# kouei/ray-tracing-in-one-weekend

Hardware: AMD Instinct MI355X
Metric: Mray/s (ray segments = closest-hit queries per second), final random-spheres scene 3840x2160 @ 500spp depth 50 (higher is better)
Workload: dtype fp32

## Files before the change

include/rt_internal.h:

```cpp
#ifndef RTOW_RT_INTERNAL_H
#define RTOW_RT_INTERNAL_H

#include "rt.h"

#ifdef __cplusplus
extern "C" {
#endif

enum { RT_OPT_INTERNAL_GRID_PHASE_X = 8, RT_OPT_INTERNAL_GRID_PHASE_Z = 9 };

enum { RT_KAT_SPHERE_HIT = 0, RT_KAT_REFLECT = 1, RT_KAT_REFRACT = 2, RT_KAT_REFLECTANCE = 3 };
int rt_device_kat(int device, int kind, const double *in, size_t n_cases, double *out);

#define RT_ACCEL_INFO_N 18
int rt_internal_accel_info(const rt_scene_view *scene, int grid_placement, double grid_scale, uint64_t *out,
                           size_t n_out);

#define RT_LAUNCH_PLAN_N 5
int rt_internal_launch_plan(const rt_params *params, double launch_samples, uint64_t *out, size_t n_out);

int rt_internal_grid_fit(const rt_scene_view *scene, const rt_camera *cam, int width, int height, double *scale,
                         double *costs, size_t n_costs, size_t *n);
int rt_internal_grid_fit_phase(const rt_scene_view *scene, const rt_camera *cam, int width, int height,
                               double phase_x, double phase_z, double *scale, double *costs, size_t n_costs,
                               size_t *n);
int rt_internal_grid_scale(rt_context *ctx, double *scale);

int rt_internal_sealed(const rt_scene_view *scene, uint8_t *out, size_t n_out);

#ifdef __cplusplus
}
#endif
#endif
```

ray-tracing-in-one-weekend_amd/csrc/rt_accel.cpp:

```cpp
#include "rt_accel.h"

#include <algorithm>
#include <cmath>
#include <cstring>
#include <vector>

namespace rtk {
namespace {

struct bvh_builder {
  struct box {
    double lo[3], hi[3];
  };
  std::vector<box> sb;
  std::vector<double> cen;
  std::vector<uint32_t> ord;
  std::vector<bvh_node> nodes;
  std::vector<int> slots;
  static constexpr int kLeaf = 2 * kLeafPairs;
  int max_leaf = kLeaf;
  double collapse_area = 0.35;
  double side_weight = 1.0;
  double grid_phase_x = 0.0, grid_phase_z = 0.0;

// ... 355 lines not shown
}

bool scene_ok(const rt_scene_view *s) {
  if (!s || (s->n && (!s->cx || !s->cy || !s->cz || !s->radius || !s->mat_kind || !s->mat_param ||
                      !s->albedo_rgb)))
    return false;
  for (uint32_t i = 0; i < s->n; ++i) {
    if (s->mat_kind[i] > RT_DIELECTRIC || !(s->radius[i] != 0.0f) || !std::isfinite(s->radius[i]) ||
        !std::isfinite(s->cx[i]) || !std::isfinite(s->cy[i]) || !std::isfinite(s->cz[i]))
      return false;
    for (int k = 0; k < 3 && s->mat_kind[i] != RT_DIELECTRIC; ++k)
      if (!(s->albedo_rgb[3 * i + k] >= 0.0f && std::isfinite(s->albedo_rgb[3 * i + k]))) return false;
  }
  return true;
}

double max_albedo(const rt_scene_view *s) {
  double a = 0.0;
  for (uint32_t i = 0; i < s->n; ++i)
    for (int k = 0; k < 3 && s->mat_kind[i] != RT_DIELECTRIC; ++k) a = std::max(a, (double)s->albedo_rgb[3 * i + k]);
  return a;
}


void build_accel(const rt_scene_view *s, const accel_options &o, accel_build &a, grid_fitter **fitter) {
  if (fitter) *fitter = nullptr;
  const uint32_t n = s->n;
  a = accel_build{};
  a.n = n;
  a.n_pad = (n + kSpherePad - 1) / kSpherePad * kSpherePad;
  a.scan_geom.assign(a.n_pad / 2, pair_geom{});
  for (uint32_t i = 0; i < a.n_pad; ++i) fill_slot(a.scan_geom[i / 2], i & 1, s, i < n ? (int)i : -1);
  a.shade.assign(n, shade_rec{});
  std::vector<uint8_t> sealed;
  sealed_spheres(s, sealed);
  for (uint32_t i = 0; i < n; ++i) {
    shade_rec &r = a.shade[i];
    std::memset(&r, 0, sizeof r);
    r.cx = s->cx[i];
    r.cy = s->cy[i];
    r.cz = s->cz[i];
    r.inv_r = 1.0f / s->radius[i];
    const bool glass = s->mat_kind[i] == RT_DIELECTRIC;
    r.ar = glass ? 1.0f : s->albedo_rgb[3 * i + 0];
    r.ag = glass ? 1.0f : s->albedo_rgb[3 * i + 1];
    r.ab = glass ? 1.0f : s->albedo_rgb[3 * i + 2];
// ... 30 lines not shown
        const double grow = std::max(1.02, 1.01 * std::sqrt((double)need / (double)lds_max));
        if (bb.grid.scale * grow > 1.6 * scale0) break;
        bb.grid.scale *= grow;
        bb.build_grid(s, bb.n_layer);
      }
      if (place != kGridCells && bb.grid.scale != scale0) {
        bb.grid.scale = scale0;
        bb.build_grid(s, bb.n_layer);
      }
    }
  }
  a.bvh_geom.assign(bb.slots.size() / 2, pair_geom{});
  for (size_t k = 0; k < bb.slots.size(); ++k) fill_slot(a.bvh_geom[k / 2], (int)(k & 1), s, bb.slots[k]);
  a.slots = bb.slots;
  a.nodes = bb.nodes;
  a.per_order = bb.per_order;
  a.oref = bb.oref;
  a.layer_mode = bb.layer_mode;
  a.layer_lo = bb.layer_lo;
  a.layer_hi = bb.layer_hi;
  a.layer_cy = bb.layer_cy;
  a.extra_pair0 = bb.extra_pair0;
  a.n_extra_pairs = bb.n_extra_pairs;
  a.grid = bb.grid;
  a.grid_placement = bb.grid.cells.empty() ? kGridGlobal : place;
  if (fitter && !bb.grid.cells.empty())
    *fitter = grid_fitter::make_from(s, o, a.grid_placement, bb.grid.scale, &bb);
}

struct grid_fitter::impl {
  std::vector<float> cx, cy, cz, radius, albedo, param;
  std::vector<uint32_t> kind;
  rt_scene_view view{};
  mutable bvh_builder bb;
  int placement = kGridGlobal;
  size_t lds_max = 0;
  double s0 = 1.0;
  bool grid_at(double scale) const {
    bb.grid.scale = scale;
    bb.build_grid(&view, bb.n_layer);
    if (bb.grid.cells.empty()) return false;
    const long long items = (long long)(bb.grid.items.size() / 4), cells = (long long)bb.grid.cells.size();
    if (placement == kGridLds)
      return items < 4096 && grid_lds_bytes(kGridLds, items, cells) <= lds_max;
    return items < 65536 && grid_lds_bytes(kGridCells, items, cells) <= lds_max;
  }
// ... 107 lines not shown
```

ray-tracing-in-one-weekend_amd/csrc/rt_accel.h:

```cpp
#ifndef RTOW_RT_ACCEL_H
#define RTOW_RT_ACCEL_H

#include <cstdint>
#include <cstring>
#include <vector>

#include "rt_internal.h"
#include "rt_layout.h"

namespace rtk {

struct accel_options {
  int bvh_leaf = 4;
  double collapse = 0.35;
  double side = 1.0;
  double grid_scale = 1.0;
  double grid_phase_x = 0.0, grid_phase_z = 0.0;
  int grid_placement = -1;
  bool wide = false;
};

struct grid_dims {
  float x0 = 0, z0 = 0, xi = 0, zi = 0, x1 = 0, z1 = 0, g = 0;
  int nx = 0, nz = 0;
// ... 4 lines not shown
  }
};
struct grid_geom : grid_dims {
  std::vector<uint32_t> cells;
  std::vector<float> items;
  bool operator==(const grid_geom &o) const {
    return grid_dims::operator==(o) && cells == o.cells && items.size() == o.items.size() &&
           (items.empty() || !std::memcmp(items.data(), o.items.data(), items.size() * sizeof(float)));
  }
};

struct accel_build {
  uint32_t n = 0, n_pad = 0;
  std::vector<pair_geom> scan_geom;
  std::vector<shade_rec> shade;
  std::vector<pair_geom> bvh_geom;
  std::vector<int> slots;
  std::vector<bvh_node> nodes;
  size_t per_order = 0;
  double oref = 64.0;
  bool layer_mode = false;
  float layer_lo = 0.0f, layer_hi = 0.0f, layer_cy = 0.0f;
  uint32_t extra_pair0 = 0, n_extra_pairs = 0;
  grid_geom grid;
  int grid_placement = kGridGlobal;
};

constexpr int kFitSteps = 30;
constexpr double kFitCellCost = 0.5;
class grid_fitter {
 public:
  static grid_fitter *make(const rt_scene_view *s, const accel_options &o, int placement, double scale0);
  ~grid_fitter();
  double choose(const rt_camera &cam, int width, int height, std::vector<std::pair<double, double>> *costs) const;
  bool build(double scale, grid_geom &out) const;
  double scale0() const;
  static grid_fitter *make_from(const rt_scene_view *s, const accel_options &o, int placement, double scale0,
                                void *builder);

 private:
  struct impl;
  impl *p_ = nullptr;
};

bool scene_ok(const rt_scene_view *s);
double max_albedo(const rt_scene_view *s);
void sealed_spheres(const rt_scene_view *s, std::vector<uint8_t> &out);
void build_accel(const rt_scene_view *s, const accel_options &o, accel_build &out, grid_fitter **fitter = nullptr);

}

#endif
```

ray-tracing-in-one-weekend_amd/csrc/rt_aov.hip:

```cpp
#include <hip/hip_runtime.h>

#include <algorithm>
#include <array>
#include <cmath>
#include <cstddef>
#include <cstdint>
#include <cstring>
#include <mutex>
#include <utility>
#include <vector>

#include "rt_aov.h"
#include "rt_device.h"
#include "rt_frame.h"

namespace rtk {

struct aov_params {
  kparams k;
  uint32_t *hits;
  int32_t *id;
  float *depth, *position, *normal, *albedo;
};
static_assert(offsetof(aov_params, k) == 0, "kernargs() reads a kparams at offset 0");
// ... 34 lines not shown
  RT_GLOBAL float *g_alb = as_global(a.albedo);
  const bool first = p.s_lo == 0;
  uint32_t hits = 0;
  int id = -1;
  float dep = 0.0f, sp[3] = {0.0f, 0.0f, 0.0f}, sn[3] = {0.0f, 0.0f, 0.0f}, sa[3] = {0.0f, 0.0f, 0.0f};
  if (!first) {
    if (a.hits) hits = g_hits[o];
    if (a.depth) dep = g_depth[o];
#pragma unroll
    for (int k = 0; k < 3; ++k) {
      if (a.position) sp[k] = g_pos[3 * o + k];
      if (a.normal) sn[k] = g_nrm[3 * o + k];
      if (a.albedo) sa[k] = g_alb[3 * o + k];
    }
  }
  if (grow < p.height) {
    const uint32_t pix = (uint32_t)grow * (uint32_t)p.width + (uint32_t)col;
    work_ctr wc;
    for (int s = p.s_lo; s < p.s_lo + p.s_cnt; ++s) {
      float ox, oy, oz, dx, dy, dz;
      const float tmin = camera_ray(p, pcg4d(pix, (uint32_t)s, 0u, p.seed32), col, grow, ox, oy, oz, dx, dy, dz);
      float walked = 0.0f;
      while (true) {
        const hit_state hs = closest_hit<OPEN, BVH, false, GRID, GP>(ox, oy, oz, dx, dy, dz, tmin, wc);
        const int best = best_of<OPEN>(hs);
        if (best < 0) break;
        const float o2 = dot3(ox, oy, oz, ox, oy, oz);
        const float ox2 = -2.0f * ox, oy2 = -2.0f * oy, oz2 = -2.0f * oz;
        const float tmax = hs.tmax;
        const bool near = near_of(hs) != 0;
        static_assert(sizeof(shade_rec) == 64, "best << 6");
        const shade_rec sr = cload_g((const RT_GLOBAL shade_rec *)((const RT_GLOBAL char *)as_global(p.shade) +
                                                                   ((uint32_t)best << 6)));
        float b;
        const float t = refine_root(sr, tmax, near, ox, oy, oz, dx, dy, dz, o2, ox2, oy2, oz2, b);
        if (b > 0.0f && t < tmin) {
          ox = fmaf(tmax, dx, ox);
          oy = fmaf(tmax, dy, oy);
          oz = fmaf(tmax, dz, oz);
          walked += tmax;
          continue;
        }
        const float px = fmaf(t, dx, ox), py = fmaf(t, dy, oy), pz = fmaf(t, dz, oz);
        const bool front = near != (sr.inv_r < 0.0f);
        const float fir = front ? sr.inv_r : -sr.inv_r;
        const float nx = (px - sr.cx) * fir, ny = (py - sr.cy) * fir, nz = (pz - sr.cz) * fir;
        ++hits;
// ... 175 lines not shown
```

ray-tracing-in-one-weekend_amd/csrc/rt_api.cpp:

```cpp
#include <hip/hip_runtime.h>

#include <algorithm>
#include <cmath>
#include <cstdint>
#include <cstring>
#include <limits>
#include <new>
#include <utility>
#include <vector>

#include "rt_internal.h"
#include "rt_accel.h"
#include "rt_frame.h"
#include "rt_layout.h"

extern "C" hipError_t rt_internal_block_order(const uint32_t *tile_cost, uint32_t blocks, uint32_t units,
                                              uint32_t *order, hipStream_t st);

struct scene_state {
  rtk::pair_geom *d_geom = nullptr;
  rtk::pair_geom *d_bvh_geom = nullptr;
  rtk::bvh_node *d_nodes = nullptr;
  int *d_orig = nullptr;
  rtk::shade_rec *d_shade = nullptr;
  uint32_t n_spheres = 0, n_pad = 0, n_nodes = 0, n_bvh_slots = 0;
  float oref2 = 0.0f;
  bool layer_mode = false;
  float layer_lo = 0.0f, layer_hi = 0.0f, layer_cy = 0.0f;
  uint32_t extra_pair0 = 0, n_extra_pairs = 0;
  uint32_t *d_grid_cells = nullptr;
  float *d_grid_items = nullptr;
  size_t cells_cap = 0, items_cap = 0;
  size_t grid_n_items = 0;
  int grid_placement = rtk::kGridGlobal;
  rtk::grid_dims grid;
  double max_albedo = 0.0;
  rtk::grid_fitter *fitter = nullptr;
  std::vector<uint64_t> fit_key;
  rtk::grid_geom fit_grid;
  bool fit_pending = false;
};

struct rt_context {
  int device = -1;
  hipStream_t stream = nullptr;
  hipEvent_t ev0 = nullptr, ev1 = nullptr;
  scene_state sc;
  hipEvent_t ev_fit = nullptr;
  bool grid_fit = true;
  bool grid_scale_set = false;
  unsigned long long *d_counters = nullptr;
  float *d_frame = nullptr;
// ... 212 lines not shown
      return RT_ERR_INVALID;
  }
}

int rt_scene_upload(rt_context *c, const rt_scene_view *s) {
  if (!c || !rtk::scene_ok(s)) return RT_ERR_INVALID;
  rtk::accel_build a;
  rtk::accel_options o = c->opt;
  o.wide = rtk::max_albedo(s) > 1.0;
  scene_state sc;
  rtk::build_accel(s, o, a, c->grid_fit && !c->grid_scale_set ? &sc.fitter : nullptr);
  sc.n_spheres = a.n;
  sc.max_albedo = rtk::max_albedo(s);
  sc.n_pad = a.n_pad;
  sc.n_nodes = (uint32_t)a.per_order;
  sc.n_bvh_slots = (uint32_t)a.slots.size();
  sc.oref2 = (float)(0.99 * a.oref * a.oref);
  sc.layer_mode = a.layer_mode;
  sc.layer_lo = a.layer_lo;
  sc.layer_cy = a.layer_cy;
  sc.layer_hi = a.layer_hi;
  sc.extra_pair0 = a.extra_pair0;
  sc.n_extra_pairs = a.n_extra_pairs;
  sc.grid = a.grid;

  hipError_t e = hipSetDevice(c->device);
  if (e == hipSuccess && c->have_done) e = hipEventSynchronize(c->ev_done);
  if (e == hipSuccess) e = hipStreamSynchronize(c->stream);
  if (e != hipSuccess) {
    release(sc);
    return hip_fail(e);
  }
  free_scene(c);
  e = upload_vec(&sc.d_geom, a.scan_geom, c->stream);
  if (e == hipSuccess) e = upload_vec(&sc.d_bvh_geom, a.bvh_geom, c->stream);
  if (e == hipSuccess) e = upload_vec(&sc.d_nodes, a.nodes, c->stream);
  if (e == hipSuccess) e = upload_vec(&sc.d_orig, a.slots, c->stream);
  if (e == hipSuccess) e = upload_vec(&sc.d_shade, a.shade, c->stream);
  if (e == hipSuccess && !a.grid.cells.empty()) {
    e = upload_vec(&sc.d_grid_cells, a.grid.cells, c->stream);
    if (e == hipSuccess) e = upload_vec(&sc.d_grid_items, a.grid.items, c->stream);
    sc.cells_cap = a.grid.cells.size();
    sc.items_cap = sc.grid_n_items = a.grid.items.size() / 4;
    sc.grid_placement = a.grid_placement;
  }
  if (e == hipSuccess) e = hipStreamSynchronize(c->stream);
// ... 41 lines not shown
void fill_kparams(const rt_context *c, const rt_camera *cam, const rt_params *prm, float *accum_rgb,
                  rtk::kparams &kp) {
  std::memset(&kp, 0, sizeof kp);
  kp.block_stride = 1;
  kp.cam = *cam;
  kp.width = prm->width;
  kp.height = prm->height;
  kp.spp = prm->spp;
  kp.max_depth = prm->max_depth;
  kp.row_block = prm->row_block;
  kp.band_stride = prm->band_stride;
  kp.band_offset = prm->band_offset;
  kp.local_rows = prm->local_rows;
  kp.tiles_x = (prm->width + rtk::kTile - 1) / rtk::kTile;
  const scene_state &s = c->sc;
  kp.n_pad = (int)s.n_pad;
  kp.n_nodes = (int)s.n_nodes;
  kp.oref2 = s.oref2;
  kp.layer = rtk::f2{s.layer_lo, s.layer_hi};
  kp.layer_mode = s.layer_mode ? 1 : 0;
  kp.layer_cy = s.layer_cy;
  kp.extra_pair0 = (int)s.extra_pair0;
  kp.n_extra_pairs = (int)s.n_extra_pairs;
  grid_kparams(s.grid, s.d_grid_cells, s.d_grid_items, s.grid_n_items, kp);
  kp.seed32 = (uint32_t)prm->seed ^ ((uint32_t)(prm->seed >> 32) * 0x9E3779B9u);
  kp.flags = prm->flags;
  kp.inv_wm1 = (float)(1.0 / (prm->width - 1));
  kp.inv_hm1 = (float)(1.0 / (prm->height - 1));
  kp.scan_geom = s.d_geom;
  kp.geom = s.d_bvh_geom;
  kp.nodes = s.d_nodes;
  kp.orig = s.d_orig;
  kp.extra_geom = s.d_bvh_geom ? s.d_bvh_geom + s.extra_pair0 : nullptr;
  kp.extra_orig = s.d_orig ? s.d_orig + 2 * (size_t)s.extra_pair0 : nullptr;
  kp.shade = s.d_shade;
  kp.out = accum_rgb;
  kp.counters = c->d_counters;
  {
    uint32_t w = (uint32_t)prm->width, sh = 0;
    while (!(w & 1u)) {
      w >>= 1;
      ++sh;
    }
    uint32_t inv = w;
    for (int k = 0; k < 5; ++k) inv *= 2u - w * inv;
    kp.wshift = sh;
    kp.winv = inv;
  }
}

int render_variant(const rt_context *c, const rt_params *prm, bool wide) {
  const bool grid = c->sc.d_grid_cells && !(prm->flags & RT_FLAG_LAYER_BVH);
  const int place = grid ? c->sc.grid_placement : rtk::kGridGlobal;
  return (wide ? rtk::kVarWide : 0) | ((prm->flags & RT_FLAG_OPEN_INTERVAL) ? rtk::kVarOpen : 0) |
         ((prm->flags & RT_FLAG_METAL_UNIT_VECTOR) ? rtk::kVarMetalUnit : 0) |
         ((prm->flags & RT_FLAG_ACCEL_BVH) ? rtk::kVarBvh : 0) |
         ((prm->flags & RT_FLAG_COUNT_WORK) ? rtk::kVarStats : 0) | (grid ? rtk::kVarGrid : 0) |
         (place << rtk::kVarPlaceShift);
}

struct launch_plan {
  long long units, ranges, chunks, entries;
};
launch_plan plan_launches(const rt_params *prm, double launch_samples) {
  const long long tiles = rt_frame_tiles(prm), blocks = rt_frame_blocks(prm);
  const bool traced = prm->spp > 0 && prm->max_depth > 0;
  const double frame_px = (double)prm->width * (double)prm->local_rows;
  const double total = traced ? frame_px * prm->spp : 0.0;
  const double budget = std::max(launch_samples, total / (double)rtk::kMaxLaunches);
  long long units = prm->units;
  if (units <= 0) {
    const bool pilot = (prm->flags & RT_FLAG_PILOT_SCHEDULE) != 0;
    units = pilot ? std::llround((double)rtk::kPilotTilesPerUnit / (double)std::max(1LL, tiles))
                  : (tiles < rtk::kSplitTiles ? rtk::kUnits : 1);
    units = std::min<long long>(std::max(units, 1LL), rtk::kUnits);
  }
  if (!traced) units = 1;
// ... 362 lines not shown
  v[7] = items;
  v[8] = cells ? rtk::grid_lds_bytes(a.grid_placement, (long long)items, (long long)cells) : 0u;
  v[9] = cells && a.grid_placement == rtk::kGridLds;
  uint64_t maxc = 0, listed = 0;
  bool start_ok = true, ring_ok = true;
  for (uint64_t i = 0; i < cells; ++i) {
    const uint32_t first = g.cells[i] >> 4, cnt = g.cells[i] & 15u;
    const uint64_t next = i + 1 < cells ? (g.cells[i + 1] >> 4) : items;
    start_ok = start_ok && first + cnt == next;
    maxc = std::max<uint64_t>(maxc, cnt);
    listed += cnt ? 1u : 0u;
    const int x = (int)(i % g.nx), z = (int)(i / g.nx);
    if (x == 0 || z == 0 || x == g.nx - 1 || z == g.nz - 1) ring_ok = ring_ok && cnt == 0;
  }
  v[10] = maxc;
  v[11] = cells ? (start_ok ? 1u : 0u) : 0u;
  v[12] = cells ? (ring_ok ? 1u : 0u) : 0u;
  v[13] = (uint64_t)(a.oref * 1000.0);
  v[14] = a.layer_mode ? (uint64_t)(2 * a.extra_pair0) : 0u;
  v[15] = listed;
  static const uint64_t kPlaceOut[3] = {RT_GRID_GLOBAL, RT_GRID_LDS, RT_GRID_CELLS_LDS};
  v[16] = cells ? kPlaceOut[a.grid_placement] : 0u;
  v[17] = (uint64_t)std::llround(g.scale * 1000.0);
  std::memcpy(out, v, std::min<size_t>(n_out, RT_ACCEL_INFO_N) * sizeof(uint64_t));
  return RT_OK;
}

int rt_internal_grid_fit(const rt_scene_view *s, const rt_camera *cam, int width, int height, double *scale,
                         double *costs, size_t n_costs, size_t *n) {
  return rt_internal_grid_fit_phase(s, cam, width, height, 0.0, 0.0, scale, costs, n_costs, n);
}

int rt_internal_grid_fit_phase(const rt_scene_view *s, const rt_camera *cam, int width, int height, double phase_x,
                               double phase_z, double *scale, double *costs, size_t n_costs, size_t *n) {
  if (!rtk::scene_ok(s) || !cam || !scale || width < 1 || height < 1 || (n_costs && !costs)) return RT_ERR_INVALID;
  if (!(phase_x >= 0.0 && phase_x < 1.0 && phase_z >= 0.0 && phase_z < 1.0)) return RT_ERR_INVALID;
  rtk::accel_options o;
  o.grid_phase_x = phase_x;
  o.grid_phase_z = phase_z;
  o.wide = rtk::max_albedo(s) > 1.0;
  rtk::accel_build a;
  rtk::grid_fitter *f = nullptr;
  rtk::build_accel(s, o, a, &f);
  *scale = 0.0;
  if (n) *n = 0;
  if (!f) return RT_OK;
// ... 60 lines not shown
```

ray-tracing-in-one-weekend_amd/csrc/rt_device.h:

```cpp
#ifndef RTOW_RT_DEVICE_H
#define RTOW_RT_DEVICE_H

#include <hip/hip_runtime.h>

#include <cstdint>

#include "rt_internal.h"
#include "rt_layout.h"
#include "rt_turn_table.h"

namespace rtk {

#ifndef RT_COUNT_ITEMS
#define RT_COUNT_ITEMS 0
#endif

enum {
  kLpStep = 0, kLpClosest, kLpExtrasLead, kLpExtrasRound, kLpGridWalk, kLpDda, kLpItem, kLpGridCand,
  kLpSky, kLpHit, kLpLamb, kLpMetal, kLpDiel, kLpCamera, kLpSkip, kLpTail, kLpRegions
};
#ifdef RT_LANE_PROFILE
__device__ unsigned long long g_lane_prof[kLpRegions * 3];
__shared__ uint32_t s_lane_prof[4][kLpRegions][3];
__device__ __forceinline__ void lane_prof(int r, bool useful) {
// ... 244 lines not shown
    const f2 gg = fma2(q[j].cz, r.oz2, fma2(q[j].cx, r.ox2, gy));
    e[j] = fma2(h[j], h[j], -gg);
    c[2 * j] = e[j].x >= q[j].ks.x;
    c[2 * j + 1] = e[j].y >= q[j].ks.y;
  }
#pragma unroll
  for (int j = 0; j < 2 * NP; ++j) any |= __builtin_amdgcn_ballot_w64(c[j]);
  if (any) {
    if (STATS) {
#pragma unroll
      for (int j = 0; j < 2 * NP; ++j) roots += __builtin_amdgcn_ballot_w64(c[j]) != 0 ? 1u : 0u;
    }
#pragma unroll
    for (int j = 0; j < NP; ++j) {
      const int s0 = slot0 + 2 * j;
      const int i0 = orig ? orig[s0] : s0;
      const int i1 = orig ? orig[s0 + 1] : s0 + 1;
      if (c[2 * j]) candidate<OPEN>(true, h[j].x, e[j].x - q[j].ks.x, tie2_of<OPEN>((uint32_t)i0), tmin, hs);
      if (c[2 * j + 1]) candidate<OPEN>(true, h[j].y, e[j].y - q[j].ks.y, tie2_of<OPEN>((uint32_t)i1), tmin, hs);
    }
  }
}

template <bool OPEN, bool STATS, bool LEAD>
__device__ __forceinline__ void scan_extras(const RT_CONST pair_geom *__restrict__ g, int slot0,
                                            const RT_CONST int *__restrict__ orig, const ray_pre &r,
                                            float tmin, hit_state &hs, uint32_t &roots) {
  float h[4], d[4];
  uint32_t t[4];
  bool c[4];
#pragma unroll
  for (int j = 0; j < 2; ++j) {
    const pair_geom q = cload(g + j);
#pragma unroll
    for (int s = 0; s < 2; ++s) {
      const float cx = s ? q.cx.y : q.cx.x, cy = s ? q.cy.y : q.cy.x, cz = s ? q.cz.y : q.cz.x;
      const float ks = s ? q.ks.y : q.ks.x;
      const float hy = fmaf(cy, r.dy.x, r.nk1.x);
      const float gy = fmaf(cy, r.oy2.x, r.o2.x);
      const float hh = fmaf(cz, r.dz.x, fmaf(cx, r.dx.x, hy));
      const float gg = fmaf(cz, r.oz2.x, fmaf(cx, r.ox2.x, gy));
      const float ee = fmaf(hh, hh, -gg);
      const int k = 2 * j + s;
      h[k] = hh;
      d[k] = ee - ks;
      c[k] = ee >= ks;
      t[k] = tie2_of<OPEN>((uint32_t)orig[slot0 + k]);
    }
  }
  constexpr int J0 = LEAD ? 1 : 0;
  if (LEAD) {
    if (__builtin_amdgcn_ballot_w64(c[0])) {
      LP(kLpExtrasLead, c[0]);
      if (STATS) ++roots;
      candidate<OPEN>(c[0], h[0], d[0], t[0], tmin, hs);
    }
  }
#pragma unroll
  for (int round = J0; round < 4; ++round) {
    float hh = h[3], dd = d[3];
    uint32_t tt = t[3];
#pragma unroll
    for (int j = 2; j >= J0; --j)
      if (c[j]) {
        hh = h[j];
        dd = d[j];
// ... 156 lines not shown
        ke = k + (ce & 15u);
      }
      uint32_t ko = k << 4;
      const uint32_t koe = ke << 4;
      if (ko != koe) do {
        grid_item<OPEN, STATS>(*(const RT_GLOBAL f4 *)((const RT_GLOBAL char *)items + ko), dx, dz, rl, tmin, hs,
                               wc);
        ko += 16;
      } while (ko != koe);
    }
    const bool sx = tmx < tmz;
    const float tnext = sx ? tmx : tmz;
    float lim;
    asm("v_min_f32 %0, %1, %2" : "=v"(lim) : "v"(tb), "v"(hs.tmax));
    const bool stop = tnext > lim;
    cell += sx ? dcx : dcz;
    tmx = sx ? tmx + tdx : tmx;
    tmz = sx ? tmz : tmz + tdz;
    asm volatile("" : "+v"(cell), "+v"(tmx), "+v"(tmz));
    if (stop) break;
  }
}

template <bool OPEN, bool BVH, bool STATS, bool GRID, int GP>
__device__ __forceinline__ hit_state closest_hit(float ox, float oy, float oz, float dx, float dy, float dz,
                                                 float tmin, work_ctr &wc) {
  const kparams p = kernargs();
  const RT_CONST pair_geom *__restrict__ scan_geom = as_const(p.scan_geom);
  const RT_CONST pair_geom *__restrict__ geom = as_const(p.geom);
  const RT_CONST bvh_node *__restrict__ nodes = as_const(p.nodes);
  const RT_CONST int *__restrict__ orig = as_const(p.orig);
  const int n_pairs = p.n_pad / 2;
  LP(kLpClosest, true);
  const float nk1 = -dot3(ox, oy, oz, dx, dy, dz);
  const float o2 = dot3(ox, oy, oz, ox, oy, oz);
  const float ox2 = -2.0f * ox, oy2 = -2.0f * oy, oz2 = -2.0f * oz;
  hit_state hs = no_hit();
  auto splat = [&]() {
    return ray_pre{{dx, dx}, {dy, dy}, {dz, dz}, {nk1, nk1}, {o2, o2}, {ox2, ox2}, {oy2, oy2}, {oz2, oz2}};
  };
  const bool scan_all = !BVH || __builtin_amdgcn_ballot_w64(o2 > p.oref2) != 0;
  if (scan_all) {
    const ray_pre rp = splat();
    for (int k = 0; k < n_pairs; k += 4)
      scan_pairs<OPEN, 4, STATS>(scan_geom + k, 2 * k, nullptr, rp, tmin, hs, wc.roots);
    if (STATS) wc.tests += 2 * n_pairs;
  } else {
    const ray_pre rp = splat();
    const float ix = __builtin_amdgcn_fmed3f(__builtin_amdgcn_rcpf(dx), -1e18f, 1e18f);
    const float iy = __builtin_amdgcn_fmed3f(__builtin_amdgcn_rcpf(dy), -1e18f, 1e18f);
    const float iz = __builtin_amdgcn_fmed3f(__builtin_amdgcn_rcpf(dz), -1e18f, 1e18f);
    const float oix = -ox * ix, oiy = -oy * iy, oiz = -oz * iz;
    auto walk_order = [&]() {
      const uint32_t half = __builtin_popcountll(__builtin_amdgcn_ballot_w64(true)) / 2;
      const int oct = (__builtin_popcountll(__builtin_amdgcn_ballot_w64(dx < 0.0f)) > half ? 1 : 0) |
                      (__builtin_popcountll(__builtin_amdgcn_ballot_w64(dy < 0.0f)) > half ? 2 : 0) |
                      (__builtin_popcountll(__builtin_amdgcn_ballot_w64(dz < 0.0f)) > half ? 4 : 0);
      return nodes + (size_t)oct * p.n_nodes;
    };
    const RT_CONST bvh_node *__restrict__ order = GRID ? nullptr : walk_order();
    if (GRID || p.layer_mode) {
      if (GRID) {
        const RT_CONST pair_geom *__restrict__ xg = as_const(p.extra_geom);
        const RT_CONST int *__restrict__ xo = as_const(p.extra_orig);
        if (p.n_extra_pairs > 0) scan_extras<OPEN, STATS, true>(xg, 0, xo, rp, tmin, hs, wc.roots);
        for (int k = 2; k < p.n_extra_pairs; k += 2)
          scan_extras<OPEN, STATS, false>(xg + k, 2 * k, xo, rp, tmin, hs, wc.roots);
      } else {
        for (int k = 0; k < p.n_extra_pairs; k += 2)
          scan_pairs<OPEN, 2, STATS>(geom + p.extra_pair0 + k, 2 * (p.extra_pair0 + k), orig, rp, tmin, hs,
                                     wc.roots);
      }
      if (STATS) wc.tests += 2 * p.n_extra_pairs;
      const f2 tyl = fma2(p.layer, f2{iy, iy}, f2{oiy, oiy});
      const float tyl_n = fmaxf(fminf(tyl.x, tyl.y), 0.0f);
      const float tyl_f = fmaxf(tyl.x, tyl.y);
      float tyl_fc = fminf(tyl_f, hs.tmax);
      if (GRID) {
        ray_pre rg = rp;
        rg.nk1.x = fmaf(p.layer_cy, dy, nk1);
        rg.o2.x = fmaf(p.layer_cy, oy2, o2);
        if (tyl_n <= tyl_fc) grid_walk<OPEN, STATS, GP>(ox, oz, ix, iz, oix, oiz, tyl_n, tyl_fc, rg, tmin, hs, wc);
        return hs;
      }
      int node = __builtin_amdgcn_ballot_w64(tyl_n <= tyl_fc) ? 0 : p.n_nodes;
      const f2 vi = {ix, iz}, vo = {oix, oiz}, va = {fabsf(ix), fabsf(iz)};
      ray_pre rl = rp;
      rl.nk1 = fma2(f2{p.layer_cy, p.layer_cy}, rp.dy, rp.nk1);
// ... 35 lines not shown
```

ray-tracing-in-one-weekend_amd/csrc/rt_kernel.hip:

```cpp
#include <hip/hip_runtime.h>

#include <algorithm>
#include <array>
#include <cmath>
#include <cstdint>
#include <type_traits>
#include <utility>

#include "rt_internal.h"
#include "rt_layout.h"
#include "rt_turn_table.h"
#include "rt_device.h"

namespace rtk {


template <bool OPEN, bool METAL_UNIT, bool BVH, bool STATS, bool GRID, int GP, bool WIDE>
__global__ __launch_bounds__(kBlock, 8) void render_kernel(const kparams p) {
  typedef typename std::conditional<WIDE, unsigned long long, uint32_t>::type sum_t;
  const int wave = __builtin_amdgcn_readfirstlane((int)threadIdx.x) >> 6;
  const unsigned entry = blockIdx.x * (unsigned)p.block_stride + (unsigned)p.block_base;
  const unsigned bid = p.block_order ? as_const(p.block_order)[entry] : entry;
  const int unit = (int)(bid % (unsigned)p.units);
  const int tile = (int)(bid / (unsigned)p.units) * kWavesPerBlock + wave;
  const int col0 = (tile % p.tiles_x) * kTile, lrow0 = (tile / p.tiles_x) * kTile;
  const uint32_t s_begin = (uint32_t)p.s_lo + (uint32_t)((uint64_t)unit * (uint32_t)p.s_cnt / (uint32_t)p.units);
  const uint32_t s_end = (uint32_t)p.s_lo + (uint32_t)((uint64_t)(unit + 1) * (uint32_t)p.s_cnt / (uint32_t)p.units);
  const uint32_t kend = (s_end > s_begin ? s_end - s_begin : 0u) << 6;
  __shared__ sum_t s_sum[3][kBlock];
  typedef uint32_t u2v __attribute__((ext_vector_type(2)));
  __shared__ u2v s_rowpix[kWavesPerBlock][kTile];
  {
    const int lane = lane_now();
    const int col = col0 + (lane & (kTile - 1));
    const int lrow = lrow0 + (lane >> 3);
    const int band = lrow / p.row_block;
    const int grow = (band * p.band_stride + p.band_offset) * p.row_block + (lrow - band * p.row_block);
    (void)col;
    if ((lane & (kTile - 1)) == 0) {
      const bool row_in = lrow < p.local_rows && grow < p.height;
// ... 38 lines not shown
    const u2v e = ((const __attribute__((address_space(3))) u2v *)(uintptr_t)rowpix_v)[slot >> 3];
    pix = e.x + (slot & (kTile - 1));
    return (slot & (kTile - 1)) < e.y;
  };
  auto pixel_cr = [&](const kparams &k, int &col, int &grow) {
    col = col0 + (int)(slot & (kTile - 1));
    grow = (int)(((pix - (uint32_t)col) >> k.wshift) * k.winv);
  };
  uint32_t knext = 64;
  bool alive = kend != 0 && p.max_depth > 0;
  bool tracing = false;
  if (alive) {
    tracing = take((uint32_t)lane_now());
    if (tracing) {
      int col, grow;
      pixel_cr(p, col, grow);
      tmin = camera_ray(p, pcg4d(pix, sample, 0u, p.seed32), col, grow, ox, oy, oz, dx, dy, dz);
    }
  }

  while (alive) {
    LP(kLpStep, tracing);
    hit_state hs = no_hit();
    if (tracing) hs = closest_hit<OPEN, BVH, STATS, GRID, GP>(ox, oy, oz, dx, dy, dz, tmin, wc);
    ++steps;
    const int best = best_of<OPEN>(hs);
    const bool miss = !tracing || best < 0;
    uint32_t kn;
    {
      const uint64_t need = __builtin_amdgcn_ballot_w64(miss);
      kn = knext + __builtin_amdgcn_mbcnt_hi((uint32_t)(need >> 32), __builtin_amdgcn_mbcnt_lo((uint32_t)need, 0u));
      knext += (uint32_t)__builtin_popcountll(need);
    }
    bool path_done = false;
    bool skipped = false;
    {
      const kparams q = kernargs();
      if (tracing) ++segs;
      if (tracing && best < 0) {
        LP(kLpSky, true);
        const float a = 0.5f * (dy + 1.0f);
        const float s0 = 1.0f - a;
        const int i = wave * 64 + (int)slot;
        float xr = thr * fmaf(a, 0.5f, s0), xg = thg * fmaf(a, 0.7f, s0), xb = thb * (s0 + a);
        if (WIDE) {
          xr = fminf(xr, q.vcap);
          xg = fminf(xg, q.vcap);
// ... 279 lines not shown
  __shared__ T thr[256];
  thr[threadIdx.x] = thr_g[threadIdx.x];
  __syncthreads();
  const uint64_t n4 = n / 4;
  const bool vec = ((uintptr_t)sums % 16 == 0) && ((uintptr_t)out % 4 == 0);
  const uint64_t stride = (uint64_t)gridDim.x * 256u;
  if (vec) {
    for (uint64_t i = (uint64_t)blockIdx.x * 256u + threadIdx.x; i < n4; i += stride) {
      const f4 v = reinterpret_cast<const f4 *>(sums)[i];
      reinterpret_cast<uint32_t *>(out)[i] =
          tone_level<FP32, T>(v.x, scale, thr) | tone_level<FP32, T>(v.y, scale, thr) << 8 |
          tone_level<FP32, T>(v.z, scale, thr) << 16 | tone_level<FP32, T>(v.w, scale, thr) << 24;
    }
  }
  for (uint64_t i = (vec ? 4 * n4 : 0) + (uint64_t)blockIdx.x * 256u + threadIdx.x; i < n; i += stride)
    out[i] = (uint8_t)tone_level<FP32, T>(sums[i], scale, thr);
}

template <int V>
void launch_variant(unsigned blocks, size_t lds, hipStream_t st, const kparams &kp) {
  constexpr bool O = V & kVarOpen, U = V & kVarMetalUnit, B = V & kVarBvh, S = V & kVarStats;
  constexpr bool G = B && (V & kVarGrid), W = V & kVarWide;
  constexpr int P = G ? ((V >> kVarPlaceShift) & 3) % 3 : kGridGlobal;
  render_kernel<O, U, B, S, G, P, W><<<blocks, kBlock, G ? lds : 0, st>>>(kp);
}
using launch_fn = void (*)(unsigned, size_t, hipStream_t, const kparams &);
template <int... V>
constexpr auto launch_table(std::integer_sequence<int, V...>) {
  return std::array<launch_fn, sizeof...(V)>{&launch_variant<V>...};
}
constexpr auto kLaunch = launch_table(std::make_integer_sequence<int, 2 * kVarWide>{});

hipError_t launch_render(int variant, unsigned blocks, size_t lds_bytes, hipStream_t st, const kparams &kp) {
  if (variant < 0 || variant >= (int)kLaunch.size()) return hipErrorInvalidValue;
  kLaunch[variant](blocks, lds_bytes, st, kp);
  return hipGetLastError();
}

hipError_t launch_finish_sums(uint32_t *frame, uint64_t n, float qinv, hipStream_t st) {
  const unsigned grid = (unsigned)std::min<uint64_t>((n + 255) / 256, 256u * 64u);
  finish_sums<<<grid, 256, 0, st>>>(frame, n, qinv);
  return hipGetLastError();
}

hipError_t launch_finish_sums_wide(const uint64_t *sums, float *frame, uint64_t n, float qinv, hipStream_t st) {
  const unsigned grid = (unsigned)std::min<uint64_t>((n + 255) / 256, 256u * 64u);
  finish_sums_wide<<<grid, 256, 0, st>>>(sums, frame, n, qinv);
  return hipGetLastError();
}

hipError_t launch_tonemap(bool fp32, const float *sums, uint64_t n, int spp, const void *thresholds,
                          uint8_t *out, hipStream_t st) {
  const unsigned grid = (unsigned)std::min<uint64_t>((n / 4 + 255) / 256 + 1, 256u * 32u);
  if (!fp32)
// ... 30 lines not shown
```

ray-tracing-in-one-weekend_amd/csrc/rt_layout.h:

```cpp
#ifndef RTOW_RT_LAYOUT_H
#define RTOW_RT_LAYOUT_H

#include <hip/hip_runtime.h>

#include <cstddef>
#include <cstdint>

#include "rt_internal.h"

namespace rtk {

constexpr int kTile = 8;
constexpr int kWavesPerBlock = 4;
constexpr int kBlock = 64 * kWavesPerBlock;
constexpr int kSpherePad = 8;
constexpr long long kSplitTiles = 12LL * 256 * 4 * 7;
constexpr long long kPilotTilesPerUnit = 16LL * 256 * 4 * 8;
constexpr int kUnits = 8;
constexpr int kCounterSlots = 32;
constexpr double kLaunchSamples = 34359738368.0;
constexpr double kMinPoolSpp = 100.0;
constexpr double kPoolSpp = 250.0;
constexpr long long kMaxLaunches = 65536;

// ... 5 lines not shown
};

struct __attribute__((aligned(32))) bvh_node {
  f2 bx, by, bz;
  int32_t skip;
  uint32_t leaf;
};
constexpr int kLeafPairs = 2;
constexpr uint32_t kTwoPairs = 1u << 31;

struct __attribute__((aligned(16))) shade_rec {
  float cx, cy, cz, inv_r;
  float ar, ag, ab, param;
  uint32_t kind;
  float radius, ks;
  float inv_param;
  float r0;
  uint32_t sealed;
  float pad1, pad2;
};

enum { kGridGlobal = 0, kGridLds = 1, kGridCells = 2 };

struct kparams {
  rt_camera cam;
  int width, height, spp, max_depth;
  int row_block, band_stride, band_offset, local_rows;
  int tiles_x, n_pad, n_nodes;
  float oref2;
  f2 layer;
  int layer_mode, extra_pair0, n_extra_pairs;
  float layer_cy;
  uint32_t seed32, flags;
  float inv_wm1, inv_hm1;
  uint32_t wshift, winv;
  int units, s_lo, s_cnt;
  int sum_atomic;
  float qscale, qinv;
  int dither, block_base;
  int block_stride;
  float vcap;
  const struct pair_geom *scan_geom;
  const struct pair_geom *geom;
  const struct bvh_node *nodes;
  const int *orig;
  const struct shade_rec *shade;
  float *out;
  unsigned long long *counters;
  const uint32_t *block_order;
  uint32_t *tile_cost;
  const uint32_t *grid_cells;
  const f4 *grid_items;
  float grid_x0, grid_z0;
  float grid_xi, grid_zi;
  float grid_x1, grid_z1, grid_g, grid_invg;
  int grid_nx, grid_nz;
  int grid_n_items, grid_n_cells;
  const struct pair_geom *extra_geom;
  const int *extra_orig;
};

__host__ __device__ constexpr size_t grid_lds_bytes(int placement, long long n_items, long long n_cells) {
  return placement == kGridLds ? (size_t)n_items * 16u + ((size_t)(n_cells + 1) * 2u + 15u) / 16u * 16u
         : placement == kGridCells ? ((size_t)(n_cells + 1) * 2u + 15u) / 16u * 16u
                                   : 0u;
}
constexpr size_t kStaticLds = 3 * kBlock * 4 + kWavesPerBlock * kTile * 8;
constexpr size_t kGridLdsMax = 160 * 1024 / 8 - kStaticLds;
constexpr size_t kGridLdsMaxWide = kGridLdsMax - 3 * kBlock * 4;

enum {
  kVarOpen = 1,
  kVarMetalUnit = 2,
  kVarBvh = 4,
  kVarStats = 8,
  kVarGrid = 16,
  kVarPlaceShift = 5,
  kVarWide = 128
};
hipError_t launch_render(int variant, unsigned blocks, size_t lds_bytes, hipStream_t st, const kparams &kp);
hipError_t launch_finish_sums(uint32_t *frame, uint64_t n, float qinv, hipStream_t st);
hipError_t launch_finish_sums_wide(const uint64_t *sums, float *frame, uint64_t n, float qinv, hipStream_t st);
hipError_t launch_tonemap(bool fp32, const float *sums, uint64_t n, int spp, const void *thresholds,
                          uint8_t *out, hipStream_t st);
hipError_t launch_kat(int kind, const double *in, int n, double *out);
hipError_t upload_turn_table();

}

#endif
```

ray-tracing-in-one-weekend_amd/rtow.py:

```python
import ctypes
import os
from dataclasses import dataclass

import numpy as np

HERE = os.path.dirname(os.path.abspath(__file__))
LIB_PATH = os.environ.get("RTOW_LIB") or os.path.join(HERE, "librtow.so")
AOV_LIB_PATH = os.path.join(HERE, "librtow_aov.so")
DENOISE_LIB_PATH = os.path.join(HERE, "librtow_denoise.so")

RT_LAMBERTIAN, RT_METAL, RT_DIELECTRIC = 0, 1, 2
RT_ERR_INVALID = -1
RT_CAMERA_CPU, RT_CAMERA_GPU = 0, 1
RT_FLAG_OPEN_INTERVAL = 1
RT_FLAG_METAL_UNIT_VECTOR = 2
RT_FLAG_GPU_SEMANTICS = 3
RT_FLAG_KEEP_COUNTERS = 1 << 8
RT_FLAG_ACCEL_BVH = 1 << 9
RT_FLAG_COUNT_WORK = 1 << 10
RT_FLAG_PILOT_SCHEDULE = 1 << 11
RT_FLAG_LAYER_BVH = 1 << 12
RT_CHUNK_SPP = 64
RT_TONEMAP_CPU, RT_TONEMAP_GPU = 0, 1
RT_KAT_SPHERE_HIT, RT_KAT_REFLECT, RT_KAT_REFRACT, RT_KAT_REFLECTANCE = 0, 1, 2, 3
# ... 482 lines not shown

def grid_fit(scene, cam, width, height, phase=(0.0, 0.0)):
    L = lib()
    L.rt_internal_grid_fit_phase.argtypes = [ctypes.c_void_p, ctypes.c_void_p, ctypes.c_int, ctypes.c_int,
                                             ctypes.c_double, ctypes.c_double,
                                             ctypes.POINTER(ctypes.c_double), ctypes.c_void_p, ctypes.c_size_t,
                                             ctypes.POINTER(ctypes.c_size_t)]
    v = scene.view()
    sc, n = ctypes.c_double(), ctypes.c_size_t()
    costs = np.zeros(2 * 64, np.float64)
    check(L.rt_internal_grid_fit_phase(ctypes.byref(v), ctypes.byref(cam), width, height, float(phase[0]),
                                       float(phase[1]), ctypes.byref(sc), costs.ctypes.data, 64,
                                       ctypes.byref(n)), "rt_internal_grid_fit_phase")
    return sc.value, [(float(costs[2 * i]), float(costs[2 * i + 1])) for i in range(min(64, n.value))]


def sealed(scene):
    v = scene.view()
    out = np.zeros(max(scene.n, 1), np.uint8)
    check(lib().rt_internal_sealed(ctypes.byref(v), out.ctypes.data, scene.n), "rt_internal_sealed")
    return out[:scene.n].astype(bool)


LAUNCH_PLAN_KEYS = ("ranges", "chunks", "units", "entries", "launches")


def launch_plan(params, launch_samples=0.0):
    out = np.zeros(len(LAUNCH_PLAN_KEYS), np.uint64)
    check(lib().rt_internal_launch_plan(ctypes.byref(params), float(launch_samples), out.ctypes.data, out.size),
          "rt_internal_launch_plan")
    return {k: int(x) for k, x in zip(LAUNCH_PLAN_KEYS, out)}


def write_ppm(path, rgb, binary=False):
    rgb = np.ascontiguousarray(rgb, dtype=np.uint8)
    h, w = rgb.shape[0], rgb.shape[1]
    fd = os.open(path, os.O_WRONLY | os.O_CREAT | os.O_TRUNC, 0o644)
    try:
        check(lib().rt_write_ppm(fd, rgb.ctypes.data, w, h, 1 if binary else 0), "rt_write_ppm")
    finally:
        os.close(fd)
```

Before: 95880.

## Specialize extras sphere test for axis-aligned and coaxial big spheres

At build time the host checks whether the first extra (large) sphere sits at x=z=0 and whether the remaining extras share one y and have z=0, which is the case for the three big spheres of the final scene. Kernel variants are templated on that fold class, so the intersection setup drops the zero terms and shares the y term across the coaxial spheres. This saves a few FMAs per ray-step in the always-scanned extras group. In exchange the number of kernel instantiations grows fourfold, which increases compile time and binary size.

```diff
diff --git a/include/rt_internal.h b/include/rt_internal.h
--- a/include/rt_internal.h
+++ b/include/rt_internal.h
@@ -12,7 +12,8 @@
 enum { RT_KAT_SPHERE_HIT = 0, RT_KAT_REFLECT = 1, RT_KAT_REFRACT = 2, RT_KAT_REFLECTANCE = 3 };
 int rt_device_kat(int device, int kind, const double *in, size_t n_cases, double *out);
 
-#define RT_ACCEL_INFO_N 18
+#define RT_ACCEL_INFO_N 36
+enum { RT_EXTRAS_AXIAL = 1, RT_EXTRAS_COAXIAL = 2 };
 int rt_internal_accel_info(const rt_scene_view *scene, int grid_placement, double grid_scale, uint64_t *out,
                            size_t n_out);
 
diff --git a/ray-tracing-in-one-weekend_amd/csrc/rt_accel.cpp b/ray-tracing-in-one-weekend_amd/csrc/rt_accel.cpp
--- a/ray-tracing-in-one-weekend_amd/csrc/rt_accel.cpp
+++ b/ray-tracing-in-one-weekend_amd/csrc/rt_accel.cpp
@@ -401,6 +401,32 @@
   return a;
 }
 
+
+int classify_extras(const rt_scene_view *s, const int *slots, size_t n_slots, float *cy) {
+  const auto bits = [](float x) {
+    uint32_t u;
+    std::memcpy(&u, &x, sizeof u);
+    return u;
+  };
+  if (cy) *cy = 0.0f;
+  if (n_slots < 4 || slots[0] < 0) return 0;
+  int cls = 0;
+  if (bits(s->cx[slots[0]]) == 0u && bits(s->cz[slots[0]]) == 0u) cls |= kFoldLead;
+  int n_rest = 0;
+  bool same = true;
+  float y = 0.0f;
+  for (int k = 1; k < 4; ++k) {
+    const int i = slots[k];
+    if (i < 0) continue;
+    if (!n_rest++) y = s->cy[i];
+    same = same && bits(s->cy[i]) == bits(y) && bits(s->cz[i]) == 0u;
+  }
+  if (n_rest && same) {
+    cls |= kFoldRest;
+    if (cy) *cy = y;
+  }
+  return cls;
+}
 
 void build_accel(const rt_scene_view *s, const accel_options &o, accel_build &a, grid_fitter **fitter) {
   if (fitter) *fitter = nullptr;
@@ -477,6 +503,9 @@
   a.layer_cy = bb.layer_cy;
   a.extra_pair0 = bb.extra_pair0;
   a.n_extra_pairs = bb.n_extra_pairs;
+  if (a.layer_mode && a.n_extra_pairs)
+    a.extras_fold = classify_extras(s, a.slots.data() + 2 * (size_t)a.extra_pair0, 2 * (size_t)a.n_extra_pairs,
+                                    &a.extras_cy);
   a.grid = bb.grid;
   a.grid_placement = bb.grid.cells.empty() ? kGridGlobal : place;
   if (fitter && !bb.grid.cells.empty())
diff --git a/ray-tracing-in-one-weekend_amd/csrc/rt_accel.h b/ray-tracing-in-one-weekend_amd/csrc/rt_accel.h
--- a/ray-tracing-in-one-weekend_amd/csrc/rt_accel.h
+++ b/ray-tracing-in-one-weekend_amd/csrc/rt_accel.h
@@ -50,6 +50,8 @@
   bool layer_mode = false;
   float layer_lo = 0.0f, layer_hi = 0.0f, layer_cy = 0.0f;
   uint32_t extra_pair0 = 0, n_extra_pairs = 0;
+  int extras_fold = 0;
+  float extras_cy = 0.0f;
   grid_geom grid;
   int grid_placement = kGridGlobal;
 };
@@ -74,6 +76,7 @@
 bool scene_ok(const rt_scene_view *s);
 double max_albedo(const rt_scene_view *s);
 void sealed_spheres(const rt_scene_view *s, std::vector<uint8_t> &out);
+int classify_extras(const rt_scene_view *s, const int *slots, size_t n_slots, float *cy);
 void build_accel(const rt_scene_view *s, const accel_options &o, accel_build &out, grid_fitter **fitter = nullptr);
 
 }
diff --git a/ray-tracing-in-one-weekend_amd/csrc/rt_aov.hip b/ray-tracing-in-one-weekend_amd/csrc/rt_aov.hip
--- a/ray-tracing-in-one-weekend_amd/csrc/rt_aov.hip
+++ b/ray-tracing-in-one-weekend_amd/csrc/rt_aov.hip
@@ -80,7 +80,16 @@
       const float tmin = camera_ray(p, pcg4d(pix, (uint32_t)s, 0u, p.seed32), col, grow, ox, oy, oz, dx, dy, dz);
       float walked = 0.0f;
       while (true) {
-        const hit_state hs = closest_hit<OPEN, BVH, false, GRID, GP>(ox, oy, oz, dx, dy, dz, tmin, wc);
+        hit_state hs;
+        const int fold = GRID ? p.extras_fold : 0;
+        if (fold == (kFoldLead | kFoldRest))
+          hs = closest_hit<OPEN, BVH, false, GRID, GP, GRID ? kFoldLead | kFoldRest : 0>(ox, oy, oz, dx, dy, dz, tmin, wc);
+        else if (fold == kFoldLead)
+          hs = closest_hit<OPEN, BVH, false, GRID, GP, GRID ? kFoldLead : 0>(ox, oy, oz, dx, dy, dz, tmin, wc);
+        else if (fold == kFoldRest)
+          hs = closest_hit<OPEN, BVH, false, GRID, GP, GRID ? kFoldRest : 0>(ox, oy, oz, dx, dy, dz, tmin, wc);
+        else
+          hs = closest_hit<OPEN, BVH, false, GRID, GP, 0>(ox, oy, oz, dx, dy, dz, tmin, wc);
         const int best = best_of<OPEN>(hs);
         if (best < 0) break;
         const float o2 = dot3(ox, oy, oz, ox, oy, oz);
diff --git a/ray-tracing-in-one-weekend_amd/csrc/rt_api.cpp b/ray-tracing-in-one-weekend_amd/csrc/rt_api.cpp
--- a/ray-tracing-in-one-weekend_amd/csrc/rt_api.cpp
+++ b/ray-tracing-in-one-weekend_amd/csrc/rt_api.cpp
@@ -28,6 +28,8 @@
   bool layer_mode = false;
   float layer_lo = 0.0f, layer_hi = 0.0f, layer_cy = 0.0f;
   uint32_t extra_pair0 = 0, n_extra_pairs = 0;
+  int extras_fold = 0;
+  float extras_cy = 0.0f;
   uint32_t *d_grid_cells = nullptr;
   float *d_grid_items = nullptr;
   size_t cells_cap = 0, items_cap = 0;
@@ -286,6 +288,8 @@
   sc.layer_hi = a.layer_hi;
   sc.extra_pair0 = a.extra_pair0;
   sc.n_extra_pairs = a.n_extra_pairs;
+  sc.extras_fold = a.extras_fold;
+  sc.extras_cy = a.extras_cy;
   sc.grid = a.grid;
 
   hipError_t e = hipSetDevice(c->device);
@@ -373,6 +377,8 @@
   kp.layer_cy = s.layer_cy;
   kp.extra_pair0 = (int)s.extra_pair0;
   kp.n_extra_pairs = (int)s.n_extra_pairs;
+  kp.extras_fold = s.extras_fold;
+  kp.extras_cy = s.extras_cy;
   grid_kparams(s.grid, s.d_grid_cells, s.d_grid_items, s.grid_n_items, kp);
   kp.seed32 = (uint32_t)prm->seed ^ ((uint32_t)(prm->seed >> 32) * 0x9E3779B9u);
   kp.flags = prm->flags;
@@ -403,7 +409,8 @@
 int render_variant(const rt_context *c, const rt_params *prm, bool wide) {
   const bool grid = c->sc.d_grid_cells && !(prm->flags & RT_FLAG_LAYER_BVH);
   const int place = grid ? c->sc.grid_placement : rtk::kGridGlobal;
-  return (wide ? rtk::kVarWide : 0) | ((prm->flags & RT_FLAG_OPEN_INTERVAL) ? rtk::kVarOpen : 0) |
+  const int fold = grid && (prm->flags & RT_FLAG_ACCEL_BVH) ? c->sc.extras_fold : 0;
+  return (fold << rtk::kVarFoldShift) | (wide ? rtk::kVarWide : 0) | ((prm->flags & RT_FLAG_OPEN_INTERVAL) ? rtk::kVarOpen : 0) |
          ((prm->flags & RT_FLAG_METAL_UNIT_VECTOR) ? rtk::kVarMetalUnit : 0) |
          ((prm->flags & RT_FLAG_ACCEL_BVH) ? rtk::kVarBvh : 0) |
          ((prm->flags & RT_FLAG_COUNT_WORK) ? rtk::kVarStats : 0) | (grid ? rtk::kVarGrid : 0) |
@@ -812,6 +819,12 @@
   static const uint64_t kPlaceOut[3] = {RT_GRID_GLOBAL, RT_GRID_LDS, RT_GRID_CELLS_LDS};
   v[16] = cells ? kPlaceOut[a.grid_placement] : 0u;
   v[17] = (uint64_t)std::llround(g.scale * 1000.0);
+  v[18] = (uint64_t)a.extras_fold;
+  uint32_t cy_bits;
+  std::memcpy(&cy_bits, &a.extras_cy, sizeof cy_bits);
+  v[19] = cy_bits;
+  for (size_t k = 0; a.layer_mode && k < 16 && k < 2 * (size_t)a.n_extra_pairs; ++k)
+    v[20 + k] = (uint64_t)(a.slots[2 * (size_t)a.extra_pair0 + k] + 1);
   std::memcpy(out, v, std::min<size_t>(n_out, RT_ACCEL_INFO_N) * sizeof(uint64_t));
   return RT_OK;
 }
diff --git a/ray-tracing-in-one-weekend_amd/csrc/rt_device.h b/ray-tracing-in-one-weekend_amd/csrc/rt_device.h
--- a/ray-tracing-in-one-weekend_amd/csrc/rt_device.h
+++ b/ray-tracing-in-one-weekend_amd/csrc/rt_device.h
@@ -290,26 +290,41 @@
   }
 }
 
-template <bool OPEN, bool STATS, bool LEAD>
+template <bool OPEN, bool STATS, bool LEAD, int FOLD = 0>
 __device__ __forceinline__ void scan_extras(const RT_CONST pair_geom *__restrict__ g, int slot0,
                                             const RT_CONST int *__restrict__ orig, const ray_pre &r,
                                             float tmin, hit_state &hs, uint32_t &roots) {
+  static_assert(LEAD || !FOLD, "only the first group is classified");
   float h[4], d[4];
   uint32_t t[4];
   bool c[4];
+  float hy1 = 0.0f, gy1 = 0.0f;
 #pragma unroll
   for (int j = 0; j < 2; ++j) {
     const pair_geom q = cload(g + j);
 #pragma unroll
     for (int s = 0; s < 2; ++s) {
+      const int k = 2 * j + s;
       const float cx = s ? q.cx.y : q.cx.x, cy = s ? q.cy.y : q.cy.x, cz = s ? q.cz.y : q.cz.x;
       const float ks = s ? q.ks.y : q.ks.x;
-      const float hy = fmaf(cy, r.dy.x, r.nk1.x);
-      const float gy = fmaf(cy, r.oy2.x, r.o2.x);
-      const float hh = fmaf(cz, r.dz.x, fmaf(cx, r.dx.x, hy));
-      const float gg = fmaf(cz, r.oz2.x, fmaf(cx, r.ox2.x, gy));
+      float hh, gg;
+      if (k == 0 && (FOLD & kFoldLead)) {
+        hh = fmaf(cy, r.dy.x, r.nk1.x);
+        gg = fmaf(cy, r.oy2.x, r.o2.x);
+      } else if (k > 0 && (FOLD & kFoldRest)) {
+        if (k == 1) {
+          hy1 = fmaf(cy, r.dy.x, r.nk1.x);
+          gy1 = fmaf(cy, r.oy2.x, r.o2.x);
+        }
+        hh = fmaf(cx, r.dx.x, hy1);
+        gg = fmaf(cx, r.ox2.x, gy1);
+      } else {
+        const float hy = fmaf(cy, r.dy.x, r.nk1.x);
+        const float gy = fmaf(cy, r.oy2.x, r.o2.x);
+        hh = fmaf(cz, r.dz.x, fmaf(cx, r.dx.x, hy));
+        gg = fmaf(cz, r.oz2.x, fmaf(cx, r.ox2.x, gy));
+      }
       const float ee = fmaf(hh, hh, -gg);
-      const int k = 2 * j + s;
       h[k] = hh;
       d[k] = ee - ks;
       c[k] = ee >= ks;
@@ -512,7 +527,7 @@
   }
 }
 
-template <bool OPEN, bool BVH, bool STATS, bool GRID, int GP>
+template <bool OPEN, bool BVH, bool STATS, bool GRID, int GP, int FOLD>
 __device__ __forceinline__ hit_state closest_hit(float ox, float oy, float oz, float dx, float dy, float dz,
                                                  float tmin, work_ctr &wc) {
   const kparams p = kernargs();
@@ -553,7 +568,7 @@
       if (GRID) {
         const RT_CONST pair_geom *__restrict__ xg = as_const(p.extra_geom);
         const RT_CONST int *__restrict__ xo = as_const(p.extra_orig);
-        if (p.n_extra_pairs > 0) scan_extras<OPEN, STATS, true>(xg, 0, xo, rp, tmin, hs, wc.roots);
+        if (p.n_extra_pairs > 0) scan_extras<OPEN, STATS, true, FOLD>(xg, 0, xo, rp, tmin, hs, wc.roots);
         for (int k = 2; k < p.n_extra_pairs; k += 2)
           scan_extras<OPEN, STATS, false>(xg + k, 2 * k, xo, rp, tmin, hs, wc.roots);
       } else {
diff --git a/ray-tracing-in-one-weekend_amd/csrc/rt_kernel.hip b/ray-tracing-in-one-weekend_amd/csrc/rt_kernel.hip
--- a/ray-tracing-in-one-weekend_amd/csrc/rt_kernel.hip
+++ b/ray-tracing-in-one-weekend_amd/csrc/rt_kernel.hip
@@ -15,7 +15,7 @@
 namespace rtk {
 
 
-template <bool OPEN, bool METAL_UNIT, bool BVH, bool STATS, bool GRID, int GP, bool WIDE>
+template <bool OPEN, bool METAL_UNIT, bool BVH, bool STATS, bool GRID, int GP, bool WIDE, int FOLD>
 __global__ __launch_bounds__(kBlock, 8) void render_kernel(const kparams p) {
   typedef typename std::conditional<WIDE, unsigned long long, uint32_t>::type sum_t;
   const int wave = __builtin_amdgcn_readfirstlane((int)threadIdx.x) >> 6;
@@ -100,7 +100,7 @@
   while (alive) {
     LP(kLpStep, tracing);
     hit_state hs = no_hit();
-    if (tracing) hs = closest_hit<OPEN, BVH, STATS, GRID, GP>(ox, oy, oz, dx, dy, dz, tmin, wc);
+    if (tracing) hs = closest_hit<OPEN, BVH, STATS, GRID, GP, FOLD>(ox, oy, oz, dx, dy, dz, tmin, wc);
     ++steps;
     const int best = best_of<OPEN>(hs);
     const bool miss = !tracing || best < 0;
@@ -426,14 +426,15 @@
   constexpr bool O = V & kVarOpen, U = V & kVarMetalUnit, B = V & kVarBvh, S = V & kVarStats;
   constexpr bool G = B && (V & kVarGrid), W = V & kVarWide;
   constexpr int P = G ? ((V >> kVarPlaceShift) & 3) % 3 : kGridGlobal;
-  render_kernel<O, U, B, S, G, P, W><<<blocks, kBlock, G ? lds : 0, st>>>(kp);
+  constexpr int F = G ? (V >> kVarFoldShift) & 3 : 0;
+  render_kernel<O, U, B, S, G, P, W, F><<<blocks, kBlock, G ? lds : 0, st>>>(kp);
 }
 using launch_fn = void (*)(unsigned, size_t, hipStream_t, const kparams &);
 template <int... V>
 constexpr auto launch_table(std::integer_sequence<int, V...>) {
   return std::array<launch_fn, sizeof...(V)>{&launch_variant<V>...};
 }
-constexpr auto kLaunch = launch_table(std::make_integer_sequence<int, 2 * kVarWide>{});
+constexpr auto kLaunch = launch_table(std::make_integer_sequence<int, kVarCount>{});
 
 hipError_t launch_render(int variant, unsigned blocks, size_t lds_bytes, hipStream_t st, const kparams &kp) {
   if (variant < 0 || variant >= (int)kLaunch.size()) return hipErrorInvalidValue;
diff --git a/ray-tracing-in-one-weekend_amd/csrc/rt_layout.h b/ray-tracing-in-one-weekend_amd/csrc/rt_layout.h
--- a/ray-tracing-in-one-weekend_amd/csrc/rt_layout.h
+++ b/ray-tracing-in-one-weekend_amd/csrc/rt_layout.h
@@ -51,6 +51,8 @@
 
 enum { kGridGlobal = 0, kGridLds = 1, kGridCells = 2 };
 
+enum { kFoldLead = RT_EXTRAS_AXIAL, kFoldRest = RT_EXTRAS_COAXIAL };
+
 struct kparams {
   rt_camera cam;
   int width, height, spp, max_depth;
@@ -87,6 +89,8 @@
   int grid_n_items, grid_n_cells;
   const struct pair_geom *extra_geom;
   const int *extra_orig;
+  int extras_fold;
+  float extras_cy;
 };
 
 __host__ __device__ constexpr size_t grid_lds_bytes(int placement, long long n_items, long long n_cells) {
@@ -105,7 +109,9 @@
   kVarStats = 8,
   kVarGrid = 16,
   kVarPlaceShift = 5,
-  kVarWide = 128
+  kVarWide = 128,
+  kVarFoldShift = 8,
+  kVarCount = 1024
 };
 hipError_t launch_render(int variant, unsigned blocks, size_t lds_bytes, hipStream_t st, const kparams &kp);
 hipError_t launch_finish_sums(uint32_t *frame, uint64_t n, float qinv, hipStream_t st);
diff --git a/ray-tracing-in-one-weekend_amd/rtow.py b/ray-tracing-in-one-weekend_amd/rtow.py
--- a/ray-tracing-in-one-weekend_amd/rtow.py
+++ b/ray-tracing-in-one-weekend_amd/rtow.py
@@ -528,6 +528,18 @@
     return out[:scene.n].astype(bool)
 
 
+RT_EXTRAS_AXIAL, RT_EXTRAS_COAXIAL = 1, 2
+
+
+def extras_info(scene):
+    v = scene.view()
+    out = np.zeros(36, np.uint64)
+    check(lib().rt_internal_accel_info(ctypes.byref(v), 0, 0.0, out.ctypes.data, out.size), "rt_internal_accel_info")
+    n = min(2 * int(out[4]), 16) if out[2] else 0
+    cy = np.array([int(out[19])], np.uint32).view(np.float32)[0]
+    return int(out[18]), cy, out[20:20 + n].astype(np.int64).astype(np.int32) - 1
+
+
 LAUNCH_PLAN_KEYS = ("ranges", "chunks", "units", "entries", "launches")
 
 
```

Result: faster. 97810, median of 6 (+2.0%).
